# tspooner/rl_markets

Measured on AMD Instinct MI355X. Metric: env-steps/sec (whole node) at 65 536 parallel books, higher is better.
Workload: dtype f64

## Files before the change

rl_markets_amd/csrc/lob_engine.hip:

```cpp
#define LOB_TU_SPLIT 1
#define LOB_TU_MAIN 1
#include <hip/hip_runtime.h>
#include <math.h>
#include <stdio.h>
#include <stdlib.h>
#include <string.h>

#include <algorithm>
#include <climits>
#include <condition_variable>
#include <initializer_list>
#include <map>
#include <mutex>
#include <string>
#include <system_error>
#include <thread>
#include <vector>

#include "lob_internal.h"
#include "lob_fast.h"
#include "lob_kernels.h"
#include "lob_launch.h"

#define HIPCHK(expr)                                                                         \
// ... 375 lines not shown
    int ndev = 0;
    if (hipGetDeviceCount(&ndev) != hipSuccess || ndev < 1 || device < 0 || device >= ndev) {
        lob_set_error("lob_create: no usable HIP device (the engine has no CPU fallback)");
        return LOB_ENODEV;
    }
    HIPCHK(hipSetDevice(device));
    lob_engine* e = new lob_engine();
    e->device = device;
    e->B = n_books;
    e->params = *p;
    e->sw = read_switches();
    {
        hipDeviceProp_t prop;
        if (hipGetDeviceProperties(&prop, device) == hipSuccess && prop.multiProcessorCount > 0) e->n_cus = prop.multiProcessorCount;
    }
#define HIPCHK_E(expr)                                                                       \
    do {                                                                                     \
        hipError_t _e = (expr);                                                              \
        if (_e != hipSuccess) {                                                              \
            lob_set_error(std::string(#expr) + ": " + hipGetErrorString(_e));                \
            lob_destroy(e);                                                                  \
            return LOB_EHIP;                                                                 \
        }                                                                                    \
    } while (0)
    HIPCHK_E(hipStreamCreate(&e->stream));
    HIPCHK_E(hipStreamCreate(&e->stream2));
    HIPCHK_E(hipEventCreateWithFlags(&e->ev_fork, hipEventDisableTiming | hipEventDisableSystemFence));
    HIPCHK_E(hipEventCreateWithFlags(&e->ev_join, hipEventDisableTiming | hipEventDisableSystemFence));
    HIPCHK_E(hipEventCreateWithFlags(&e->ev_stagger, hipEventDisableTiming | hipEventDisableSystemFence));
    HIPCHK_E(hipEventCreateWithFlags(&e->ev_rest_go, hipEventDisableTiming | hipEventDisableSystemFence));
    HIPCHK_E(hipEventCreateWithFlags(&e->ev_rest_done, hipEventDisableTiming | hipEventDisableSystemFence));
    if (hipHostMalloc((void**)&e->rest_hint, LOB_HINT_RING * sizeof(u64), hipHostMallocMapped) == hipSuccess) {
        memset(e->rest_hint, 0, LOB_HINT_RING * sizeof(u64));
        if (hipHostGetDevicePointer((void**)&e->rest_hint_dev, e->rest_hint, 0) != hipSuccess) e->rest_hint_dev = nullptr;
    } else e->rest_hint = nullptr;
    if (!e->rest_hint_dev && e->rest_hint) { hipHostFree(e->rest_hint); e->rest_hint = nullptr; }
    for (int i = 0; i < LOB_HINT_RING && e->rest_hint; i++) HIPCHK_E(hipEventCreateWithFlags(&e->hint_ev[i], hipEventDisableTiming));

    DevParams& P = e->P;
    memset(&P, 0, sizeof P);
    P.D = p->depth; P.T = p->max_trades; P.W = lob_rec_words(p->depth, p->max_trades); P.Wd = drec_words(p->depth, p->max_trades); P.V = p->n_vars;
    for (int i = 0; i < LOB_MAX_VARS; i++) P.vars[i] = p->vars[i];
    lobh::TickTable tt;
    lobh::build_tick_table(p->market, tt);
    P.n_bands = tt.n;
    for (int i = 0; i < LOB_MAX_BANDS; i++) { P.band_lb[i] = tt.lb[i]; P.band_tick[i] = tt.tick[i]; P.band_cum[i] = tt.cum[i]; P.band_pt[i] = tt.pt[i]; P.band_pp[i] = tt.pp[i]; }
    P.open_ms = p->market.open_ms; P.close_ms = p->market.close_ms;
    P.order_size = p->order_size; P.reward_measure = p->reward_measure;
    P.pos_lb = p->pos_lb; P.pos_ub = p->pos_ub;
    P.damping_factor = p->damping_factor; P.pos_weight = p->pos_weight; P.trd_weight = p->trd_weight; P.pnl_weight = p->pnl_weight;
    P.target_price = p->target_price; P.quote_mode = p->quote_mode;
    P.ewma_alpha = 2.0 / ((double)(size_t)p->lb_rsi + 1.0);
    P.M = p->memory_size;
    P.w0 = p->group_weights[0]; P.w1 = p->group_weights[1]; P.w2 = p->group_weights[2];
    P.gamma = p->gamma; P.alpha = p->alpha; P.epsilon = p->epsilon;
    P.policy = p->policy; P.tau = p->tau; P.beta = p->beta;
    P.trace_rate = trace_rate;
    for (int k = 0; k <= LOB_TRACE_GENS; k++) P.trace_pow[k] = trace_pow[k];
    P.trace_kmax = trace_kmax;
    P.trace_gens = P.trace_kmax <= 32 ? 32 : LOB_TRACE_GENS;
    P.r_learn = p->algo >= LOB_ALGO_R_LEARN;
    P.algo = p->algo == LOB_ALGO_R_LEARN ? LOB_ALGO_QLAMBDA : p->algo == LOB_ALGO_ONLINE_R_LEARN ? LOB_ALGO_SARSA
             : p->algo == LOB_ALGO_DOUBLE_R_LEARN ? LOB_ALGO_DOUBLE_Q : p->algo;
    P.theta_private = p->theta_mode == LOB_THETA_PRIVATE;
    e->plan = plan_paths(P, n_books, e->n_cus, e->sw);
    P.combine = e->plan.combine;
    P.memo = e->plan.memo;
    P.carry_verdicts = e->plan.carry_verdicts;
    P.sarsa_lanes = e->plan.sarsa_lanes;
    P.epi_epoch = 0;
    P.seed = p->seed; P.book_id_offset = p->book_id_offset;
    P.exp_learn_first = e->sw.exp_learn_first ? 1 : 0;

    DevState& S = e->S;
    memset(&S, 0, sizeof S);
    const size_t B = (size_t)n_books;
    S.B = n_books; S.D = P.D; S.T = P.T; S.W = P.W;
    int rc = LOB_OK;
    auto alloc = [&](auto* ptr, size_t count) { if (rc == LOB_OK) rc = dev_alloc(e, ptr, count); };
#define X(t, n) alloc(&S.n, B);
    LOB_ENV_FIELDS(X)
#undef X
    alloc(&S.hdr, B);
    auto alloc_rm = [&](RMPtrs& r, int w) {
        r.w = w;
        alloc(&r.ring, B * w); alloc(&r.cnt, B); alloc(&r.head, B); alloc(&r.sum, B); alloc(&r.mean, B); alloc(&r.s, B);
    };
    auto alloc_acc = [&](AccPtrs& r, int w) {
        r.w = w;
        alloc(&r.ring, B * w); alloc(&r.cnt, B); alloc(&r.head, B); alloc(&r.sum, B);
    };
    alloc_rm(S.f_midprice, p->lb_mpm);
    alloc_rm(S.f_volatility, p->lb_vlt);
    alloc_rm(S.f_ask_tx, p->lb_svl);
    alloc_rm(S.f_bid_tx, p->lb_svl);
    alloc_rm(S.spread_window, p->lb_spread);
    alloc_rm(S.pnl_ups, p->lb_pnl);
    alloc_rm(S.pnl_downs, p->lb_pnl);
    alloc_rm(S.tp_mp, p->lb_target);
    alloc_acc(S.f_vwap_numer, p->lb_vwap);
    alloc_acc(S.f_vwap_denom, p->lb_vwap);
    alloc(&S.meta, B); alloc(&S.prep, B); alloc(&S.ewma_up, B); alloc(&S.ewma_down, B); alloc(&S.tp_val, B); alloc(&S.persist, B * LOB_PERSIST_N);
    alloc(&S.k_stop, B); alloc(&S.vars, B * 3 * 16); alloc(&S.qs_last, B * LOB_N_ACTIONS); alloc(&S.tr_idx, B * (size_t)P.trace_gens * 32);
    alloc(&S.tr_alive, B * (size_t)P.trace_gens); alloc(&S.theta, (size_t)P.M * (P.theta_private ? B : 1));
    alloc(&S.theta_nz, LOB_NZ_NWORDS(P.M) * (P.theta_private ? B : 1));
    if (P.algo == LOB_ALGO_DOUBLE_Q) {
        alloc(&S.theta_b, (size_t)P.M * (P.theta_private ? B : 1)); alloc(&S.theta_b_nz, LOB_NZ_NWORDS(P.M) * (P.theta_private ? B : 1));
        alloc(&S.qs_last_b, B * LOB_N_ACTIONS); alloc(&S.mt_state, B * LOB_MT_N); alloc(&S.mt_idx, B);
    }
    {
        const bool rl = P.r_learn != 0;
        const size_t nr = rl ? (P.theta_private ? B : 1) : 1;
        alloc(&S.rho, nr); alloc(&S.rho_inc, nr); alloc(&S.rho_cnt, nr); alloc(&S.rl_t, rl ? B : 1);
    }
    alloc(&S.tr_sig, B * (size_t)P.trace_gens * 4); alloc(&S.tr_cbslot, B * (size_t)P.trace_gens);
    {
        int slots = 2048;
        while ((size_t)slots < 8 * B && slots < (1 << 22)) slots <<= 1;
        if (e->sw.cb_slots) slots = e->sw.cb_slots;
        S.cb_slots = slots;
        alloc(&S.cb_key, (size_t)slots); alloc(&S.cb_ident, (size_t)slots * 8);
        S.cb_reps = e->sw.acc_reps ? e->sw.acc_reps : P.memo ? 8 : 1;
        alloc(&S.cb_acc, (size_t)S.cb_reps * slots * 2); alloc(&S.cb_touch, (size_t)slots); alloc(&S.cb_list, 2 * (size_t)slots);
        S.cb_segs = std::min(2048, slots / 4);
        alloc(&S.cb_count, 2 * (size_t)S.cb_segs);
        if (rc == LOB_OK && hipMemsetAsync(S.cb_key, 0xff, (size_t)slots * 8, e->stream) != hipSuccess) rc = LOB_EHIP;
        if (e->plan.dense_ids) {
            alloc(&S.cb_dense, (size_t)slots); alloc(&S.cb_free, (size_t)LOB_CBD_CAP); alloc(&S.cb_free_n, 16);
            alloc(&S.tr_cbd, B * (size_t)P.trace_gens); alloc(&S.cb_part, (size_t)LOB_ACD_MAX_BLOCKS * LOB_CBD_CAP);
            alloc(&S.cb_red, (size_t)LOB_ACD_GROUPS * LOB_CBD_CAP);
            if (rc == LOB_OK && hipMemsetAsync(S.cb_dense, 0xff, (size_t)slots * 4, e->stream) != hipSuccess) rc = LOB_EHIP;
            if (rc == LOB_OK && hipMemsetAsync(S.tr_cbd, 0xff, B * (size_t)P.trace_gens * 8, e->stream) != hipSuccess) rc = LOB_EHIP;
            if (rc == LOB_OK) {
                std::vector<i32> fl(LOB_CBD_CAP), fn(16);
                const int per = LOB_CBD_CAP / 8;
                int have = per;
                if (e->sw.cbd_ids) have = e->sw.cbd_ids / 8;
                S.cb_ids = have * 8;
                for (int x = 0; x < 8; x++) {
                    for (int i = 0; i < have; i++) fl[(size_t)x * per + i] = (have - 1 - i) * 8 + x;
                    fn[2 * x] = have;
                    fn[2 * x + 1] = have;
                }
                if (hipMemcpyAsync(S.cb_free, fl.data(), fl.size() * 4, hipMemcpyHostToDevice, e->stream) != hipSuccess ||
                    hipMemcpyAsync(S.cb_free_n, fn.data(), fn.size() * 4, hipMemcpyHostToDevice, e->stream) != hipSuccess ||
                    hipStreamSynchronize(e->stream) != hipSuccess) rc = LOB_EHIP;
            }
            if (rc == LOB_OK && hipFuncSetAttribute((const void*)accumulate_dense_kernel, hipFuncAttributeMaxDynamicSharedMemorySize, (int)acd_lds_bytes()) != hipSuccess) {
                lob_set_error("hipFuncSetAttribute(accumulate_dense_kernel: dynamic LDS)");
                rc = LOB_EHIP;
            }
        }
    }
    {
        S.mk_slots = 1 << 16;
        const size_t ms = (size_t)S.mk_slots;
        alloc(&S.mk_hash, ms); alloc(&S.mk_ident, ms * 4); alloc(&S.mk_stamp, ms); alloc(&S.mk_list, 2 * ms); alloc(&S.mk_count, 2);
        alloc(&S.mk_rec, 2 * ms * LOB_MK_REC);
        if (P.memo && P.algo == LOB_ALGO_DOUBLE_Q) alloc(&S.mk_rec_b, 2 * ms * LOB_MK_REC);
        alloc(&S.mk_tiles, P.memo ? ms * LOB_N_ACTIONS * 32 : 1); alloc(&S.mk_tiles_ok, ms); alloc(&S.mk_marked, ms); alloc(&S.mk_marklist, ms);
        alloc(&S.mk_markcount, 1); alloc(&S.tr_list, B); alloc(&S.tr_list_n, 2); alloc(&S.tr_list2, B); alloc(&S.tr_list2_n, 2);
        alloc(&S.acc_list, B); alloc(&S.acc_list_n, 2); alloc(&S.acc_pend, B); alloc(&S.dir_list, P.combine ? B * (size_t)P.trace_gens : 1);
        alloc(&S.dir_list_n, 2); alloc(&S.mk_slot, B); alloc(&S.mk_slot_last, B);
        if (rc == LOB_OK && hipMemsetAsync(S.mk_hash, 0xff, ms * 8, e->stream) != hipSuccess) rc = LOB_EHIP;
        if (rc == LOB_OK && hipMemsetAsync(S.mk_slot, 0xff, B * 4, e->stream) != hipSuccess) rc = LOB_EHIP;
        if (rc == LOB_OK && hipMemsetAsync(S.mk_slot_last, 0xff, B * 4, e->stream) != hipSuccess) rc = LOB_EHIP;
        const bool sl = P.sarsa_lanes != 0;
        S.ow_slots = sl ? 1 << 25 : 1;
        S.amb_cap = sl ? (int)std::min<long long>((long long)P.M, 1 << 18) : 1;
        if (sl && e->sw.ow_slots) S.ow_slots = e->sw.ow_slots;
        if (sl && e->sw.amb_cap) S.amb_cap = e->sw.amb_cap;
        alloc(&S.tr_mslot, sl ? B * (size_t)P.trace_gens : 1); alloc(&S.ow_tab, (size_t)S.ow_slots);
        alloc(&S.amb_bits, sl ? (size_t)P.M / 32 + 1 : 1); alloc(&S.amb_new, 2 * (size_t)S.amb_cap); alloc(&S.amb_new_n, 2); alloc(&S.amb_flag, 1);
        alloc(&S.mk_amb, sl ? ms * LOB_N_ACTIONS : 1); alloc(&S.mk_all, sl ? ms : 1); alloc(&S.mk_all_n, 1);
        if (rc == LOB_OK && hipMemsetAsync(S.tr_mslot, 0xff, (sl ? B * (size_t)P.trace_gens : 1) * 4, e->stream) != hipSuccess) rc = LOB_EHIP;
        if (rc == LOB_OK && hipMemsetAsync(S.ow_tab, 0xff, (size_t)S.ow_slots * 8, e->stream) != hipSuccess) rc = LOB_EHIP;
    }
    {
        int cs = 5;
        while ((((size_t)P.M >> cs) + 31) / 32 > 20480) cs++;
        P.cshift = cs;
        const size_t cwords = (((size_t)P.M >> cs) + 32) / 32;
        P.cwords4 = (int)((cwords + 3) / 4);
        alloc(&S.theta_nzx, P.memo ? (size_t)P.M / 32 + 1 : 1); alloc(&S.theta_nzc, (size_t)P.cwords4 * 4);
// ... 1711 lines not shown
```

rl_markets_amd/csrc/lob_env.h:

```cpp
#ifndef LOB_ENV_H
#define LOB_ENV_H

#include <hip/hip_runtime.h>

#include "lob_internal.h"
#include "lob_state.h"

LOB_HD int drec_pad4(int n) { return (n + 3) & ~3; }
LOB_HD int drec_words(int D, int T) { return 4 + 4 * drec_pad4(D) + drec_pad4(2 * T); }
LOB_HD int drec_ask_px(int, int) { return 4; }
LOB_HD int drec_ask_vol(int D, int) { return 4 + drec_pad4(D); }
LOB_HD int drec_bid_px(int D, int) { return 4 + 2 * drec_pad4(D); }
LOB_HD int drec_bid_vol(int D, int) { return 4 + 3 * drec_pad4(D); }
LOB_HD int drec_trades(int D, int) { return 4 + 4 * drec_pad4(D); }
LOB_HD void drec_from_abi(const uint32_t* src, int D, int T, uint32_t* dst) {
    const int Wd = drec_words(D, T);
    for (int i = 0; i < Wd; i++) dst[i] = 0;
    dst[0] = src[LOB_REC_TIME];
    dst[1] = src[LOB_REC_FLAGS];
    for (int l = 0; l < D; l++) {
        dst[drec_ask_px(D, T) + l] = src[lob_rec_ask_px(D, T) + l];
        dst[drec_ask_vol(D, T) + l] = src[lob_rec_ask_vol(D, T) + l];
        dst[drec_bid_px(D, T) + l] = src[lob_rec_bid_px(D, T) + l];
        dst[drec_bid_vol(D, T) + l] = src[lob_rec_bid_vol(D, T) + l];
// ... 1412 lines not shown

__device__ inline void persist_io(const DevState& S, int b, bool save) {
    int i = 0;
    const int B = S.B;
#define X(n)                                                                                   \
    if (save) { S.persist[(size_t)(i + 0) * B + b] = S.n.sum[b]; S.persist[(size_t)(i + 1) * B + b] = S.n.mean[b]; S.persist[(size_t)(i + 2) * B + b] = S.n.s[b]; } \
    else { S.n.sum[b] = S.persist[(size_t)(i + 0) * B + b]; S.n.mean[b] = S.persist[(size_t)(i + 1) * B + b]; S.n.s[b] = S.persist[(size_t)(i + 2) * B + b]; }   \
    i += 3;
    X(f_midprice) X(f_volatility) X(f_ask_tx) X(f_bid_tx) X(spread_window) X(tp_mp)
#undef X
#define X(n)                                                            \
    if (save) S.persist[(size_t)i * B + b] = S.n.sum[b];                \
    else S.n.sum[b] = S.persist[(size_t)i * B + b];                     \
    i += 1;
    X(f_vwap_numer) X(f_vwap_denom)
#undef X
    if (save) {
        S.persist[(size_t)(i + 0) * B + b] = S.ewma_up[b];
        S.persist[(size_t)(i + 1) * B + b] = S.ewma_down[b];
        S.persist[(size_t)(i + 2) * B + b] = S.tp_val[b];
    } else {
        S.ewma_up[b] = S.persist[(size_t)(i + 0) * B + b];
        S.ewma_down[b] = S.persist[(size_t)(i + 1) * B + b];
        S.tp_val[b] = S.persist[(size_t)(i + 2) * B + b];
    }
}

__device__ inline void prepass_begin(const EnvCtx& c, PrepState& st, BookMeta& M) {
    const DevParams& P = c.P;
    const DevState& S = c.S;
    const int b = c.b;
    MarketR m;
    m.cursor = 0; m.time_ms = 0; m.rec_cur = -1; m.rec_last = -1;
    m.ap0 = m.bp0 = m.lap0 = m.lbp0 = 0.0;
    m.a_tv = m.b_tv = 0;
    m.a_obsval = m.b_obsval = 0.0; m.a_obsvol = m.b_obsvol = 0;
    m.ewma_up = S.ewma_up[b]; m.ewma_down = S.ewma_down[b]; m.tp_val = S.tp_val[b];
    m.records = 0;
#define X(n) S.n.cnt[b] = 0;
    LOB_ROLLING_MEANS(X)
    LOB_ACCUMULATORS(X)
#undef X
    M.n_track = 0; M.k_warm = -1; M.init_ok = 0; M.complete = 0; M._pad = 0;
    M.ex_first = -1; M.ex_cur = -1; M.ex_last = -1; M.ex_time = 0; M.ex_records = 0;
    bool ok = true;
    while (ok && !is_open(P, m.time_ms)) ok = mk_update_book_profiles(c, m);
    M.rec_cur0 = m.rec_cur; M.rec_last0 = m.rec_last; M.time0 = m.time_ms;
    M.mid0 = (m.ap0 + m.bp0) / 2.0; M.mid_prev0 = (m.lap0 + m.lbp0) / 2.0;
    if (!ok) { M.ex_cur = m.rec_cur; M.ex_last = m.rec_last; M.ex_time = m.time_ms; M.complete = 1; }
    st.cursor = m.cursor; st.time_ms = m.time_ms; st.rec_cur = m.rec_cur; st.rec_last = m.rec_last;
    st.ap0 = m.ap0; st.bp0 = m.bp0; st.lap0 = m.lap0; st.lbp0 = m.lbp0;
    st.a_tv = m.a_tv; st.b_tv = m.b_tv;
    st.ewma_up = m.ewma_up; st.ewma_down = m.ewma_down; st.tp_val = m.tp_val;
    st.records = m.records;
    st.k = 0;
    st.prev_first = m.rec_cur;
}

__device__ inline void prepass_begin_books(const EnvCtx& c, PrepState& st, BookMeta& M) {
    const DevParams& P = c.P;
    MarketR m;
    m.cursor = 0; m.time_ms = 0; m.rec_cur = -1; m.rec_last = -1;
    m.ap0 = m.bp0 = m.lap0 = m.lbp0 = 0.0;
    m.a_tv = m.b_tv = 0;
    m.a_obsval = m.b_obsval = 0.0; m.a_obsvol = m.b_obsvol = 0;
    m.ewma_up = m.ewma_down = m.tp_val = 0.0;
    m.records = 0;
    M.n_track = 0; M.k_warm = -1; M.init_ok = 0; M.complete = 0; M._pad = 0;
    M.ex_first = -1; M.ex_cur = -1; M.ex_last = -1; M.ex_time = 0; M.ex_records = 0;
    bool ok = true;
    while (ok && !is_open(P, m.time_ms)) ok = mk_update_book_profiles(c, m);
    M.rec_cur0 = m.rec_cur; M.rec_last0 = m.rec_last; M.time0 = m.time_ms;
    M.mid0 = (m.ap0 + m.bp0) / 2.0; M.mid_prev0 = (m.lap0 + m.lbp0) / 2.0;
    if (!ok) { M.ex_cur = m.rec_cur; M.ex_last = m.rec_last; M.ex_time = m.time_ms; M.complete = 1; }
    st.cursor = m.cursor; st.time_ms = m.time_ms; st.rec_cur = m.rec_cur; st.rec_last = m.rec_last;
    st.ap0 = m.ap0; st.bp0 = m.bp0; st.lap0 = m.lap0; st.lbp0 = m.lbp0;
    st.a_tv = m.a_tv; st.b_tv = m.b_tv;
    st.ewma_up = st.ewma_down = st.tp_val = 0.0;
    st.records = m.records;
    st.k = 0;
    st.prev_first = m.rec_cur;
}

template <int TM>
__device__ inline void prepass_run(const EnvCtx& c, PrepState& st, BookMeta& M, int k_stop, bool write_track) {
    const DevParams& P = c.P;
    const DevState& S = c.S;
    const int b = c.b, B = S.B;
    MarketR m;
    m.cursor = st.cursor; m.time_ms = st.time_ms; m.rec_cur = st.rec_cur; m.rec_last = st.rec_last;
    m.ap0 = st.ap0; m.bp0 = st.bp0; m.lap0 = st.lap0; m.lbp0 = st.lbp0;
    m.a_tv = st.a_tv; m.b_tv = st.b_tv;
    m.a_obsval = m.b_obsval = 0.0; m.a_obsvol = m.b_obsvol = 0;
    m.ewma_up = st.ewma_up; m.ewma_down = st.ewma_down; m.tp_val = st.tp_val;
    m.records = st.records;
    int k = st.k;
    int prev_first = st.prev_first;
    RMReg w_mid, w_vol, w_spr, w_tp, w_atx, w_btx;
    AccReg w_vn, w_vd;
    rm_load(S.f_midprice, b, w_mid); rm_load(S.f_volatility, b, w_vol); rm_load(S.spread_window, b, w_spr);
    rm_load(S.tp_mp, b, w_tp); rm_load(S.f_ask_tx, b, w_atx); rm_load(S.f_bid_tx, b, w_btx);
    acc_load(S.f_vwap_numer, b, w_vn); acc_load(S.f_vwap_denom, b, w_vd);
#ifndef LOB_PRE_TOUCH
#define LOB_PRE_TOUCH 0
#endif
#if LOB_PRE_TOUCH
    PreRow<TM> R0;
    uint32_t nt[4] = {0u, 0u, 0u, 0u};
#else
    PreRow<TM> R0, R1;
#endif
    i32 t1 = 0, t2 = 0;
    bool piped = false;
    int band_px = 0, band_tk = 0;
    rm_prep(S.f_midprice, B, b, w_mid); rm_prep(S.f_volatility, B, b, w_vol); rm_prep(S.spread_window, B, b, w_spr);
    rm_prep(S.tp_mp, B, b, w_tp); rm_prep(S.f_ask_tx, B, b, w_atx); rm_prep(S.f_bid_tx, B, b, w_btx);
    acc_prep(S.f_vwap_numer, B, b, w_vn); acc_prep(S.f_vwap_denom, B, b, w_vd);
    while (!M.complete && k < k_stop) {
        const int first = m.cursor;
#if LOB_PRE_TOUCH
        {
            const int last = c.n_ev() - 1;
            const uint32_t* r2 = c.row(first + 2 < last ? first + 2 : last);
            const int wl = P.Wd - 1;
            nt[0] = r2[0]; nt[1] = r2[16 < wl ? 16 : wl]; nt[2] = r2[32 < wl ? 32 : wl]; nt[3] = r2[wl];
        }
        pre_row_issue<TM>(c, first, R0);
        if (!piped) t1 = pre_row_time(c, first + 1);
#else
        if (!piped) { pre_row_issue<TM>(c, first, R0); t1 = pre_row_time(c, first + 1); }
        pre_row_issue<TM>(c, first + 1, R1);
        t2 = pre_row_time(c, first + 2);
#endif
        if (first < c.n_ev() && (R0.hdr.y & LOB_EVT_FLAG_TAS_DRY)) {
            M.ex_first = -1; M.ex_cur = m.rec_cur; M.ex_last = m.rec_last; M.ex_time = m.time_ms; M.ex_records = 0;
            M.complete = 1;
            break;
        }
        f64 tp[TM];
        i64 tv[TM];
        if (prev_first + 1 == first) {
#pragma unroll
            for (int i = 0; i < TM; i++) { tp[i] = 0.0; tv[i] = 0; }
            int ntr = 0;
            merge_trade_slots<TM>(c, R0.tr, ntr, tp, tv);
        } else {
            load_trades<TM>(c, prev_first + 1, first, tp, tv);
        }
        prev_first = first;
        const f64 mp = (m.ap0 + m.bp0) / 2.0;
        m.a_obsval = 0.0; m.a_obsvol = 0; m.b_obsval = 0.0; m.b_obsvol = 0;
#pragma unroll
        for (int i = 0; i < TM; i++) {
            if (i >= P.T || tv[i] <= 0) continue;
            if (tp[i] < mp) continue;
            m.a_obsval += tp[i] * (f64)tv[i];
            m.a_obsvol += tv[i];
        }
#pragma unroll
        for (int ii = 0; ii < TM; ii++) {
            const int i = TM - 1 - ii;
            if (i >= P.T || tv[i] <= 0) continue;
            if (tp[i] > mp) continue;
            m.b_obsval += tp[i] * (f64)tv[i];
            m.b_obsvol += tv[i];
        }
        const i64 rec0 = m.records;
        if (!mk_update_book_profiles_pre<TM>(c, m, R0, t1)) {
            M.ex_first = first; M.ex_cur = m.rec_cur; M.ex_last = m.rec_last; M.ex_time = m.time_ms;
            M.ex_records = m.records - rec0;
            M.complete = 1;
            break;
        }
        if (m.lap0 == 0.0 || m.lbp0 == 0.0) c.err(LOB_ERR_UNDEF_PRICE);
        const f64 mid = (m.ap0 + m.bp0) / 2.0, lmid = (m.lap0 + m.lbp0) / 2.0;
        const int tick_ap0 = lobh::to_ticks_hint((*c.tk), m.ap0, band_px), tick_bp0 = lobh::to_ticks_hint((*c.tk), m.bp0, band_px);
        const i64 mpt = (i64)lobh::to_ticks_hint((*c.tk), mid, band_px);
        const f64 mpm = mid - lmid, sp = m.ap0 - m.bp0;
        rm_apply_reg(S.f_midprice, B, b, w_mid, (f64)mpt);
        rm_apply_reg(S.f_volatility, B, b, w_vol, (f64)mpt);
        acc_apply_reg(S.f_vwap_numer, B, b, w_vn, m.a_obsval + m.b_obsval);
        acc_apply_reg(S.f_vwap_denom, B, b, w_vd, (f64)(m.a_obsvol + m.b_obsvol));
        rm_apply_reg(S.spread_window, B, b, w_spr, 0.0 > sp ? 0.0 : sp);
        f64 micro;
        {
            f64 div = (f64)(m.a_tv + m.b_tv);
            f64 mpm_a = (f64)m.a_tv * m.bp0, mpm_b = m.ap0 * (f64)m.b_tv;
            micro = (mpm_a + mpm_b) / div;
        }
        rm_apply_reg(S.tp_mp, B, b, w_tp, P.target_price == LOB_TP_MICROPRICE ? micro : mid);
        m.tp_val = w_tp.mean;
        {
            f64 up = 0.0 > mpm ? 0.0 : mpm;
            f64 dn = fabs(0.0 < mpm ? 0.0 : mpm);
            m.ewma_up = (P.ewma_alpha * up) + ((1 - P.ewma_alpha) * m.ewma_up);
            m.ewma_down = (P.ewma_alpha * dn) + ((1 - P.ewma_alpha) * m.ewma_down);
        }
        rm_apply_reg(S.f_ask_tx, B, b, w_atx, (f64)m.a_obsvol);
        rm_apply_reg(S.f_bid_tx, B, b, w_btx, (f64)m.b_obsvol);
        rm_prep(S.f_midprice, B, b, w_mid); rm_prep(S.f_volatility, B, b, w_vol); rm_prep(S.spread_window, B, b, w_spr);
        rm_prep(S.tp_mp, B, b, w_tp); rm_prep(S.f_ask_tx, B, b, w_atx); rm_prep(S.f_bid_tx, B, b, w_btx);
        acc_prep(S.f_vwap_numer, B, b, w_vn); acc_prep(S.f_vwap_denom, B, b, w_vd);

        if (write_track) {
            Track t;
            t.rec_first = first; t.rec_last = m.rec_cur; t.time_ms = m.time_ms;
            t.tick_ap0 = tick_ap0; t.tick_bp0 = tick_bp0;
            {
                int ntr = 0;
#pragma unroll
                for (int i = 0; i < TM; i++) ntr += (i < P.T && tv[i] > 0) ? 1 : 0;
                t.info = (ntr < 2 ? ntr : 2) | (ntr <= 2 ? LOB_TRK_TRADES_OK : 0);
                t.tr_px[0] = (f32)tp[0]; t.tr_vol[0] = tv[0];
                t.tr_px[1] = TM > 1 ? (f32)tp[TM > 1 ? 1 : 0] : 0.0f; t.tr_vol[1] = TM > 1 ? tv[TM > 1 ? 1 : 0] : 0;
                t.bap = (f32)m.ap0; t.bbp = (f32)m.bp0;
            }
            t.mid = mid; t.tp_val = m.tp_val; t.spread_mean = w_spr.mean;
            t.a_tv = m.a_tv; t.b_tv = m.b_tv;
            t.mv[LOB_MV_SPD] = (f32)ulb((f64)(tick_ap0 - tick_bp0), 0.0, 20.0);
            {
                const f64 front = (f64)mpt;
                i32 bi = w_mid.head - w_mid.cnt + 1;
                if (bi < 0) bi += S.f_midprice.w;
                const f64 back = w_mid.cnt == S.f_midprice.w ? w_mid.old : S.f_midprice.ring[(size_t)bi * B + b];
                t.mv[LOB_MV_MPM] = (f32)ulb((f64)(lobh::to_ticks_hint((*c.tk), front, band_tk) - lobh::to_ticks_hint((*c.tk), back, band_tk)), -10.0, 10.0);
            }
            {
                f64 v_a = (f64)m.a_tv, v_b = (f64)m.b_tv;
                t.mv[LOB_MV_IMB] = (f32)((v_a + v_b) > 0 ? 5 * (v_b - v_a) / (v_b + v_a) : 0.0);
                f64 q_a = w_atx.sum, q_b = w_btx.sum;
                t.mv[LOB_MV_SVL] = (f32)((q_a + q_b) > 0 ? 5 * (q_b - q_a) / (q_a + q_b) : 0.0);
            }
            {
                f64 var = w_vol.s / (f64)(w_vol.cnt - 1);
                f64 sd = var > 0 ? sqrt(var) : 0.0;
                t.mv[LOB_MV_VOL] = (f32)ulb(5.0 * sd, 0.0, 10.0);
                f64 u = m.ewma_up, d = m.ewma_down;
                t.mv[LOB_MV_RSI] = (f32)((u + d) != 0.0 ? 5.0 * (u - d) / (u + d) : 0.0);
                f64 vw = w_vn.sum / w_vd.sum;
                t.mv[LOB_MV_VWAP] = (f32)ulb(vw / w_spr.mean, -10.0, 10.0);
                t.mv[7] = 0.0f;
            }
            c.track_w(k) = t;
            if (M.k_warm < 0 && w_atx.cnt == S.f_ask_tx.w && w_btx.cnt == S.f_bid_tx.w && w_vn.cnt == S.f_vwap_numer.w &&
                w_vd.cnt == S.f_vwap_denom.w && w_vol.cnt == S.f_volatility.w && w_mid.cnt == S.f_midprice.w &&
                w_tp.cnt == S.tp_mp.w && w_spr.cnt == S.spread_window.w)
                M.k_warm = k + 1;
        }
        if (k + 1 == M.k_warm) prev_first = m.rec_cur;
        k++;
        piped = m.cursor == first + 1;
#if LOB_PRE_TOUCH
        t2 = (i32)nt[0];
        asm volatile("" ::"v"(nt[1]), "v"(nt[2]), "v"(nt[3]));
        if (piped) t1 = t2;
#else
        if (piped) { R0 = R1; t1 = t2; }
#endif
    }
    rm_store(S.f_midprice, b, w_mid); rm_store(S.f_volatility, b, w_vol); rm_store(S.spread_window, b, w_spr);
    rm_store(S.tp_mp, b, w_tp); rm_store(S.f_ask_tx, b, w_atx); rm_store(S.f_bid_tx, b, w_btx);
    acc_store(S.f_vwap_numer, b, w_vn); acc_store(S.f_vwap_denom, b, w_vd);
    st.cursor = m.cursor; st.time_ms = m.time_ms; st.rec_cur = m.rec_cur; st.rec_last = m.rec_last;
    st.ap0 = m.ap0; st.bp0 = m.bp0; st.lap0 = m.lap0; st.lbp0 = m.lbp0;
    st.a_tv = m.a_tv; st.b_tv = m.b_tv;
    st.ewma_up = m.ewma_up; st.ewma_down = m.ewma_down; st.tp_val = m.tp_val;
    st.records = m.records;
    st.k = k;
    st.prev_first = prev_first;
    S.ewma_up[b] = m.ewma_up; S.ewma_down[b] = m.ewma_down; S.tp_val[b] = m.tp_val;
    if (write_track) {
        M.n_track = k;
        M.init_ok = M.k_warm > 0 ? 1 : 0;
    }
}


__device__ inline void lds_block_barrier() {
    __builtin_amdgcn_fence(__ATOMIC_RELEASE, "workgroup", "local");
    __builtin_amdgcn_s_barrier();
    __builtin_amdgcn_fence(__ATOMIC_ACQUIRE, "workgroup", "local");
}
struct PreXch {
    i64 mpt[64], a_obsvol[64], b_obsvol[64], a_tv[64], b_tv[64];
    f64 sp[64], mpm[64], tp_in[64], obsval[64];
    i32 spd[64], live[64];
    i32 go, _pad;
};
template <int TM>
__device__ inline void prepass_books_role(const DevParams* Pp, const DevState* Sp, int b, const uint32_t* rows, const TickLds* tk, PrepState* stp, BookMeta* Mp,
                                                int k_stop, bool on, PreXch* xch, int lane) {
    const DevParams& P = *Pp;
    const DevState& S = *Sp;
    const EnvCtx c(P, S, b, tk, rows);
    PrepState& st = *stp;
    BookMeta& M = *Mp;
    MarketR m;
    m.cursor = st.cursor; m.time_ms = st.time_ms; m.rec_cur = st.rec_cur; m.rec_last = st.rec_last;
    m.ap0 = st.ap0; m.bp0 = st.bp0; m.lap0 = st.lap0; m.lbp0 = st.lbp0;
    m.a_tv = st.a_tv; m.b_tv = st.b_tv;
    m.a_obsval = m.b_obsval = 0.0; m.a_obsvol = m.b_obsvol = 0;
    m.ewma_up = m.ewma_down = m.tp_val = 0.0;
    m.records = st.records;
    int k = st.k;
    int prev_first = st.prev_first;
    PreRow<TM> R0;
    uint32_t nt[4] = {0u, 0u, 0u, 0u};
    i32 t1 = 0;
    bool piped = false;
    int band_px = 0;
    int w_max = S.f_midprice.w;
    {
        const int ws[] = {S.f_volatility.w, S.f_ask_tx.w, S.f_bid_tx.w, S.spread_window.w, S.tp_mp.w, S.f_vwap_numer.w, S.f_vwap_denom.w};
        for (int w : ws) w_max = w > w_max ? w : w_max;
    }
#pragma unroll 1
    for (int it = 0;; it++) {
        PreXch& X = xch[it & 1];
        int live = 0;
        if (on && !M.complete && k < k_stop) {
            do {
                const int first = m.cursor;
                {
                    const int last = c.n_ev() - 1;
                    const uint32_t* r2 = c.row(first + 2 < last ? first + 2 : last);
                    const int wl = P.Wd - 1;
                    nt[0] = r2[0]; nt[1] = r2[16 < wl ? 16 : wl]; nt[2] = r2[32 < wl ? 32 : wl]; nt[3] = r2[wl];
                }
                pre_row_issue<TM>(c, first, R0);
                if (!piped) t1 = pre_row_time(c, first + 1);
                if (first < c.n_ev() && (R0.hdr.y & LOB_EVT_FLAG_TAS_DRY)) {
                    M.ex_first = -1; M.ex_cur = m.rec_cur; M.ex_last = m.rec_last; M.ex_time = m.time_ms; M.ex_records = 0;
                    M.complete = 1;
                    break;
                }
                f64 tp[TM];
                i64 tv[TM];
                if (prev_first + 1 == first) {
#pragma unroll
                    for (int i = 0; i < TM; i++) { tp[i] = 0.0; tv[i] = 0; }
                    int ntr = 0;
                    merge_trade_slots<TM>(c, R0.tr, ntr, tp, tv);
                } else {
                    load_trades<TM>(c, prev_first + 1, first, tp, tv);
                }
// ... 174 lines not shown
```

rl_markets_amd/csrc/lob_state.h:

```cpp
#ifndef LOB_STATE_H
#define LOB_STATE_H

#include <stdint.h>

#include "../../include/lob_engine.h"

typedef long long i64;
typedef unsigned long long u64;
typedef int i32;
typedef double f64;
typedef float f32;

#if defined(__HIP_DEVICE_COMPILE__)
template <class T> __device__ __forceinline__ T* lob_g(T* p) {
    return (T*)(__attribute__((address_space(1))) T*)(unsigned long long)p;
}
#else
template <class T> inline T* lob_g(T* p) { return p; }
#endif

template <class T> struct GP {
    T* p;
    __host__ __device__ __forceinline__ operator T*() const { return lob_g(p); }
    __host__ __device__ __forceinline__ T* operator->() const { return lob_g(p); }
// ... 103 lines not shown
    f64 ap0, bp0, lap0, lbp0;
    i64 a_tv, b_tv;
    f64 ewma_up, ewma_down, tp_val;
    i64 records;
    i32 k;
    i32 prev_first;
};

struct __attribute__((aligned(64))) LHdr {
    i32 done;
    i32 time_ms;
    i32 slot_cur;
    i32 zero_mask;
    i32 action;
    i32 stepped;
    i32 tr_head;
    i32 tr_n;
    u64 rng_ctr;
    f64 reward;
    f64 td;
    f64 upd;
};

#define LOB_CBD_CAP 16384
#define LOB_ACD_MAX_BLOCKS 256
#define LOB_ACD_MARK 0x7ff4000000000001ull
#define LOB_ML_BLOCKS 256
#define LOB_ML_ROWS 8192
#define LOB_PERSIST_N 32
#define LOB_PROF_N 32
#define LOB_MK_REC 10
#define LOB_MK_PROBES 16
#define LOB_HL_CAP 23
#define LOB_HL_ROW 24
#define LOB_HL_MAX 35
#define LOB_HL_REC 36
#define LOB_VD_STRIDE 72
#define LOB_NZ_SHIFT 3
#define LOB_NZ_WORD(i) ((i) >> (LOB_NZ_SHIFT + 5))
#define LOB_NZ_BIT(i) (1u << (((i) >> LOB_NZ_SHIFT) & 31))
#define LOB_NZ_NWORDS(M) ((((size_t)(M) >> LOB_NZ_SHIFT) >> 5) + 1)
#define LOB_NZ_WORDS 256
#define LOB_NZ_FILTER 128
#define LOB_NZ_NEW_MAX 256

struct RMPtrs {
    GP<f64> ring;
    GP<i32> cnt;
    GP<i32> head;
    GP<f64> sum;
    GP<f64> mean;
    GP<f64> s;
    i32 w;
};
struct AccPtrs {
    GP<f64> ring;
    GP<i32> cnt;
    GP<i32> head;
    GP<f64> sum;
    i32 w;
};

struct DevState {
    i32 B;
    i32 D, T, W;
    i32 n_events;
    GP<const uint32_t> records;
    GP<const i64> rec_phase;
    GP<const i32> rec_len;
    __device__ __forceinline__ i32 events_of(int b) const { return rec_len ? rec_len[b] : n_events; }

#define X(t, n) GP<t> n;
    LOB_ENV_FIELDS(X)
#undef X
#define X(n) RMPtrs n;
    LOB_ROLLING_MEANS(X)
#undef X
#define X(n) AccPtrs n;
    LOB_ACCUMULATORS(X)
#undef X

    GP<Track> track;
    i32 track_len, track_mask;
    GP<BookMeta> meta;
    GP<PrepState> prep;
    GP<f64> ewma_up;
    GP<f64> ewma_down;
    GP<f64> tp_val;
    GP<f64> persist;
    GP<i32> k_stop;

    GP<LHdr> hdr;
    GP<f32> vars;
    GP<f64> qs_last;
    GP<i32> tr_idx;
    GP<uint32_t> tr_alive;

    GP<f64> theta;
    GP<f64> theta_b;
    GP<uint32_t> theta_b_nz;
    GP<f64> qs_last_b;
    GP<u64> mt_state;
    GP<i32> mt_idx;
    GP<i32> tr_sig;
    GP<i32> tr_cbslot;
    GP<i32> tr_mslot;
    GP<u64> cb_key;
    GP<i32> cb_ident;
    GP<f64> cb_acc;
    GP<uint32_t> cb_touch;
    GP<i32> cb_list;
    GP<i32> cb_count;
    i32 cb_slots;
    i32 cb_reps;
    i32 cb_segs;
    i32 cb_par;
    GP<i32> cb_dense;
    GP<i32> cb_free;
    GP<i32> cb_free_n;
    GP<u64> tr_cbd;
    GP<f64> cb_part;
    GP<f64> cb_red;
    i32 cb_ids;
    i32 cb_dense_on;
    GP<uint16_t> verdict;
    GP<uint16_t> verdict_b;
    GP<i32> nz_new;
    GP<i32> nz_epoch;
    GP<uint32_t> theta_nz;
    GP<u64> mk_hash;
    GP<i32> mk_ident;
    GP<i32> mk_stamp;
    GP<i32> mk_list;
    GP<i32> mk_count;
    GP<f64> mk_rec;
    GP<f64> mk_rec_b;
    GP<i32> mk_tiles;
    GP<i32> mk_tiles_ok;
    GP<uint32_t> mk_marked;
    GP<i32> mk_marklist;
    GP<i32> mk_markcount;
    GP<u64> ow_tab;
    i32 ow_slots;
    GP<uint32_t> amb_bits;
    GP<i32> amb_new;
    GP<i32> amb_new_n;
    i32 amb_cap;
    GP<i32> amb_flag;
    GP<uint32_t> mk_amb;
    GP<i32> mk_all;
    GP<i32> mk_all_n;
    GP<i32> mk_slot;
    GP<i32> mk_slot_last;
    i32 mk_slots;
    GP<uint32_t> theta_nzx;
    GP<uint32_t> theta_nzc;
    GP<uint32_t> theta_nzd;
    GP<const uint32_t> nzd_terms;
    GP<i32> tr_list;
    GP<i32> tr_list_n;
    GP<i32> tr_list2;
    GP<i32> tr_list2_n;
    GP<i32> acc_list;
    GP<i32> acc_list_n;
    GP<uint8_t> acc_pend;
    GP<i32> dir_list;
// ... 89 lines not shown
```

Baseline: 288.9 million.

## Index prepass rolling-window rings by step with power-of-two mask and shared midprice ring

Rolling-window rings used in the prepass are now sized to a common power of two and addressed by step index `k & mask`. This replaces per-window head/count bookkeeping in registers. The volatility window reuses the midprice ring because both push the same value, which removes one ring's storage and writes. Evicted values are prefetched one step ahead, and warm-up is detected with a single comparison against the largest window. Head and count are reconstructed from k only at the end, so any other code that reads these rings with the old head-based layout could disagree.

```diff
diff --git a/rl_markets_amd/csrc/lob_engine.hip b/rl_markets_amd/csrc/lob_engine.hip
--- a/rl_markets_amd/csrc/lob_engine.hip
+++ b/rl_markets_amd/csrc/lob_engine.hip
@@ -481,24 +481,34 @@
     LOB_ENV_FIELDS(X)
 #undef X
     alloc(&S.hdr, B);
-    auto alloc_rm = [&](RMPtrs& r, int w) {
+    int pre_len = 1;
+    for (int w : {p->lb_mpm, p->lb_vlt, p->lb_svl, p->lb_spread, p->lb_target, p->lb_vwap})
+        while (pre_len < w) pre_len *= 2;
+    S.pre_mask = pre_len - 1;
+    auto alloc_rm = [&](RMPtrs& r, int w, int ring_len) {
         r.w = w;
-        alloc(&r.ring, B * w); alloc(&r.cnt, B); alloc(&r.head, B); alloc(&r.sum, B); alloc(&r.mean, B); alloc(&r.s, B);
+        if (ring_len) alloc(&r.ring, B * ring_len);
+        alloc(&r.cnt, B); alloc(&r.head, B); alloc(&r.sum, B); alloc(&r.mean, B); alloc(&r.s, B);
     };
-    auto alloc_acc = [&](AccPtrs& r, int w) {
+    auto alloc_acc = [&](AccPtrs& r, int w, int ring_len) {
         r.w = w;
-        alloc(&r.ring, B * w); alloc(&r.cnt, B); alloc(&r.head, B); alloc(&r.sum, B);
+        alloc(&r.ring, B * ring_len); alloc(&r.cnt, B); alloc(&r.head, B); alloc(&r.sum, B);
     };
-    alloc_rm(S.f_midprice, p->lb_mpm);
-    alloc_rm(S.f_volatility, p->lb_vlt);
-    alloc_rm(S.f_ask_tx, p->lb_svl);
-    alloc_rm(S.f_bid_tx, p->lb_svl);
-    alloc_rm(S.spread_window, p->lb_spread);
-    alloc_rm(S.pnl_ups, p->lb_pnl);
-    alloc_rm(S.pnl_downs, p->lb_pnl);
-    alloc_rm(S.tp_mp, p->lb_target);
-    alloc_acc(S.f_vwap_numer, p->lb_vwap);
-    alloc_acc(S.f_vwap_denom, p->lb_vwap);
+    alloc_rm(S.f_midprice, p->lb_mpm, pre_len);
+#ifdef LOB_EXPERIMENTS
+    alloc_rm(S.f_volatility, p->lb_vlt, pre_len);
+#else
+    alloc_rm(S.f_volatility, p->lb_vlt, 0);
+    S.f_volatility.ring = S.f_midprice.ring.p;
+#endif
+    alloc_rm(S.f_ask_tx, p->lb_svl, pre_len);
+    alloc_rm(S.f_bid_tx, p->lb_svl, pre_len);
+    alloc_rm(S.spread_window, p->lb_spread, pre_len);
+    alloc_rm(S.pnl_ups, p->lb_pnl, p->lb_pnl);
+    alloc_rm(S.pnl_downs, p->lb_pnl, p->lb_pnl);
+    alloc_rm(S.tp_mp, p->lb_target, pre_len);
+    alloc_acc(S.f_vwap_numer, p->lb_vwap, pre_len);
+    alloc_acc(S.f_vwap_denom, p->lb_vwap, pre_len);
     alloc(&S.meta, B); alloc(&S.prep, B); alloc(&S.ewma_up, B); alloc(&S.ewma_down, B); alloc(&S.tp_val, B); alloc(&S.persist, B * LOB_PERSIST_N);
     alloc(&S.k_stop, B); alloc(&S.vars, B * 3 * 16); alloc(&S.qs_last, B * LOB_N_ACTIONS); alloc(&S.tr_idx, B * (size_t)P.trace_gens * 32);
     alloc(&S.tr_alive, B * (size_t)P.trace_gens); alloc(&S.theta, (size_t)P.M * (P.theta_private ? B : 1));
diff --git a/rl_markets_amd/csrc/lob_env.h b/rl_markets_amd/csrc/lob_env.h
--- a/rl_markets_amd/csrc/lob_env.h
+++ b/rl_markets_amd/csrc/lob_env.h
@@ -1518,6 +1518,37 @@
     st.prev_first = m.rec_cur;
 }
 
+struct PreRM { f64 sum, mean, s, old; };
+struct PreAcc { f64 sum, old; };
+__device__ inline size_t pre_slot(int k, int mask, int B) { return (size_t)(k & mask) * B; }
+__device__ inline void pre_rm_load(const RMPtrs& r, int b, PreRM& g) { g.sum = r.sum[b]; g.mean = r.mean[b]; g.s = r.s[b]; g.old = 0.0; }
+__device__ inline void pre_rm_push(PreRM& g, f64 val, int k, int w) {
+    g.sum += val;
+    const f64 n = (f64)((k < w ? k : w) + 1);
+    const f64 old_mean = g.mean;
+    g.mean += (val - g.mean) / n;
+    g.s += (val - g.mean) * (val - old_mean);
+    if (k >= w) {
+        g.sum -= g.old;
+        const f64 n2 = (f64)w;
+        const f64 old_mean2 = g.mean;
+        g.mean -= (g.old - g.mean) / n2;
+        g.s -= (g.old - g.mean) * (g.old - old_mean2);
+    }
+}
+__device__ inline void pre_acc_push(PreAcc& g, f64 val, int k, int w) {
+    g.sum += val;
+    if (k >= w) g.sum -= g.old;
+}
+__device__ inline void pre_cnt_head(i32* cnt, i32* head, int b, int k, int w) {
+    cnt[b] = k < w ? k : w;
+    if (k > 0) head[b] = (k - 1) % w;
+}
+__device__ inline void pre_rm_store(const RMPtrs& r, int b, const PreRM& g, int k) {
+    r.sum[b] = g.sum; r.mean[b] = g.mean; r.s[b] = g.s;
+    pre_cnt_head(r.cnt, r.head, b, k, r.w);
+}
+
 template <int TM>
 __device__ inline void prepass_run(const EnvCtx& c, PrepState& st, BookMeta& M, int k_stop, bool write_track) {
     const DevParams& P = c.P;
@@ -1532,11 +1563,20 @@
     m.records = st.records;
     int k = st.k;
     int prev_first = st.prev_first;
-    RMReg w_mid, w_vol, w_spr, w_tp, w_atx, w_btx;
-    AccReg w_vn, w_vd;
-    rm_load(S.f_midprice, b, w_mid); rm_load(S.f_volatility, b, w_vol); rm_load(S.spread_window, b, w_spr);
-    rm_load(S.tp_mp, b, w_tp); rm_load(S.f_ask_tx, b, w_atx); rm_load(S.f_bid_tx, b, w_btx);
-    acc_load(S.f_vwap_numer, b, w_vn); acc_load(S.f_vwap_denom, b, w_vd);
+    PreRM w_mid, w_vol, w_spr, w_tp, w_atx, w_btx;
+    PreAcc w_vn, w_vd;
+    pre_rm_load(S.f_midprice, b, w_mid); pre_rm_load(S.f_volatility, b, w_vol); pre_rm_load(S.spread_window, b, w_spr);
+    pre_rm_load(S.tp_mp, b, w_tp); pre_rm_load(S.f_ask_tx, b, w_atx); pre_rm_load(S.f_bid_tx, b, w_btx);
+    w_vn.sum = S.f_vwap_numer.sum[b]; w_vd.sum = S.f_vwap_denom.sum[b];
+    const int pm = S.pre_mask;
+    f64* const r_px = S.f_midprice.ring + b; f64* const r_spr = S.spread_window.ring + b; f64* const r_tp = S.tp_mp.ring + b;
+    f64* const r_atx = S.f_ask_tx.ring + b; f64* const r_btx = S.f_bid_tx.ring + b;
+    f64* const r_vn = S.f_vwap_numer.ring + b; f64* const r_vd = S.f_vwap_denom.ring + b;
+    const int wl_mid = S.f_midprice.w, wl_vol = S.f_volatility.w, wl_spr = S.spread_window.w, wl_tp = S.tp_mp.w, wl_svl = S.f_ask_tx.w,
+              wl_vwap = S.f_vwap_numer.w;
+    int w_max = wl_mid;
+    w_max = wl_vol > w_max ? wl_vol : w_max; w_max = wl_spr > w_max ? wl_spr : w_max; w_max = wl_tp > w_max ? wl_tp : w_max;
+    w_max = wl_svl > w_max ? wl_svl : w_max; w_max = wl_vwap > w_max ? wl_vwap : w_max;
 #ifndef LOB_PRE_TOUCH
 #define LOB_PRE_TOUCH 0
 #endif
@@ -1549,9 +1589,13 @@
     i32 t1 = 0, t2 = 0;
     bool piped = false;
     int band_px = 0, band_tk = 0;
-    rm_prep(S.f_midprice, B, b, w_mid); rm_prep(S.f_volatility, B, b, w_vol); rm_prep(S.spread_window, B, b, w_spr);
-    rm_prep(S.tp_mp, B, b, w_tp); rm_prep(S.f_ask_tx, B, b, w_atx); rm_prep(S.f_bid_tx, B, b, w_btx);
-    acc_prep(S.f_vwap_numer, B, b, w_vn); acc_prep(S.f_vwap_denom, B, b, w_vd);
+#define LOB_PRE_FETCH(kk)                                                                                                   \
+    w_mid.old = r_px[pre_slot((kk) - wl_mid, pm, B)]; w_vol.old = r_px[pre_slot((kk) - wl_vol, pm, B)];                        \
+    w_spr.old = r_spr[pre_slot((kk) - wl_spr, pm, B)]; w_tp.old = r_tp[pre_slot((kk) - wl_tp, pm, B)];                         \
+    { const size_t o = pre_slot((kk) - wl_svl, pm, B); w_atx.old = r_atx[o]; w_btx.old = r_btx[o]; }                          \
+    { const size_t o = pre_slot((kk) - wl_vwap, pm, B); w_vn.old = r_vn[o]; w_vd.old = r_vd[o]; }
+    LOB_PRE_FETCH(k)
+    f64 mid_cur = (m.ap0 + m.bp0) / 2.0;
     while (!M.complete && k < k_stop) {
         const int first = m.cursor;
 #if LOB_PRE_TOUCH
@@ -1584,7 +1628,7 @@
             load_trades<TM>(c, prev_first + 1, first, tp, tv);
         }
         prev_first = first;
-        const f64 mp = (m.ap0 + m.bp0) / 2.0;
+        const f64 mp = mid_cur;
         m.a_obsval = 0.0; m.a_obsvol = 0; m.b_obsval = 0.0; m.b_obsvol = 0;
 #pragma unroll
         for (int i = 0; i < TM; i++) {
@@ -1610,21 +1654,24 @@
         }
         if (m.lap0 == 0.0 || m.lbp0 == 0.0) c.err(LOB_ERR_UNDEF_PRICE);
         const f64 mid = (m.ap0 + m.bp0) / 2.0, lmid = (m.lap0 + m.lbp0) / 2.0;
+        mid_cur = mid;
         const int tick_ap0 = lobh::to_ticks_hint((*c.tk), m.ap0, band_px), tick_bp0 = lobh::to_ticks_hint((*c.tk), m.bp0, band_px);
         const i64 mpt = (i64)lobh::to_ticks_hint((*c.tk), mid, band_px);
         const f64 mpm = mid - lmid, sp = m.ap0 - m.bp0;
-        rm_apply_reg(S.f_midprice, B, b, w_mid, (f64)mpt);
-        rm_apply_reg(S.f_volatility, B, b, w_vol, (f64)mpt);
-        acc_apply_reg(S.f_vwap_numer, B, b, w_vn, m.a_obsval + m.b_obsval);
-        acc_apply_reg(S.f_vwap_denom, B, b, w_vd, (f64)(m.a_obsvol + m.b_obsvol));
-        rm_apply_reg(S.spread_window, B, b, w_spr, 0.0 > sp ? 0.0 : sp);
+        const size_t slot = pre_slot(k, pm, B);
+        r_px[slot] = (f64)mpt;
+        pre_rm_push(w_mid, (f64)mpt, k, wl_mid);
+        pre_rm_push(w_vol, (f64)mpt, k, wl_vol);
+        pre_acc_push(w_vn, r_vn[slot] = m.a_obsval + m.b_obsval, k, wl_vwap);
+        pre_acc_push(w_vd, r_vd[slot] = (f64)(m.a_obsvol + m.b_obsvol), k, wl_vwap);
+        pre_rm_push(w_spr, r_spr[slot] = 0.0 > sp ? 0.0 : sp, k, wl_spr);
         f64 micro;
         {
             f64 div = (f64)(m.a_tv + m.b_tv);
             f64 mpm_a = (f64)m.a_tv * m.bp0, mpm_b = m.ap0 * (f64)m.b_tv;
             micro = (mpm_a + mpm_b) / div;
         }
-        rm_apply_reg(S.tp_mp, B, b, w_tp, P.target_price == LOB_TP_MICROPRICE ? micro : mid);
+        pre_rm_push(w_tp, r_tp[slot] = P.target_price == LOB_TP_MICROPRICE ? micro : mid, k, wl_tp);
         m.tp_val = w_tp.mean;
         {
             f64 up = 0.0 > mpm ? 0.0 : mpm;
@@ -1632,11 +1679,9 @@
             m.ewma_up = (P.ewma_alpha * up) + ((1 - P.ewma_alpha) * m.ewma_up);
             m.ewma_down = (P.ewma_alpha * dn) + ((1 - P.ewma_alpha) * m.ewma_down);
         }
-        rm_apply_reg(S.f_ask_tx, B, b, w_atx, (f64)m.a_obsvol);
-        rm_apply_reg(S.f_bid_tx, B, b, w_btx, (f64)m.b_obsvol);
-        rm_prep(S.f_midprice, B, b, w_mid); rm_prep(S.f_volatility, B, b, w_vol); rm_prep(S.spread_window, B, b, w_spr);
-        rm_prep(S.tp_mp, B, b, w_tp); rm_prep(S.f_ask_tx, B, b, w_atx); rm_prep(S.f_bid_tx, B, b, w_btx);
-        acc_prep(S.f_vwap_numer, B, b, w_vn); acc_prep(S.f_vwap_denom, B, b, w_vd);
+        pre_rm_push(w_atx, r_atx[slot] = (f64)m.a_obsvol, k, wl_svl);
+        pre_rm_push(w_btx, r_btx[slot] = (f64)m.b_obsvol, k, wl_svl);
+        LOB_PRE_FETCH(k + 1)
 
         if (write_track) {
             Track t;
@@ -1656,9 +1701,7 @@
             t.mv[LOB_MV_SPD] = (f32)ulb((f64)(tick_ap0 - tick_bp0), 0.0, 20.0);
             {
                 const f64 front = (f64)mpt;
-                i32 bi = w_mid.head - w_mid.cnt + 1;
-                if (bi < 0) bi += S.f_midprice.w;
-                const f64 back = w_mid.cnt == S.f_midprice.w ? w_mid.old : S.f_midprice.ring[(size_t)bi * B + b];
+                const f64 back = k + 1 >= wl_mid ? w_mid.old : r_px[0];
                 t.mv[LOB_MV_MPM] = (f32)ulb((f64)(lobh::to_ticks_hint((*c.tk), front, band_tk) - lobh::to_ticks_hint((*c.tk), back, band_tk)), -10.0, 10.0);
             }
             {
@@ -1668,7 +1711,7 @@
                 t.mv[LOB_MV_SVL] = (f32)((q_a + q_b) > 0 ? 5 * (q_b - q_a) / (q_a + q_b) : 0.0);
             }
             {
-                f64 var = w_vol.s / (f64)(w_vol.cnt - 1);
+                f64 var = w_vol.s / (f64)((k + 1 < wl_vol ? k + 1 : wl_vol) - 1);
                 f64 sd = var > 0 ? sqrt(var) : 0.0;
                 t.mv[LOB_MV_VOL] = (f32)ulb(5.0 * sd, 0.0, 10.0);
                 f64 u = m.ewma_up, d = m.ewma_down;
@@ -1678,10 +1721,7 @@
                 t.mv[7] = 0.0f;
             }
             c.track_w(k) = t;
-            if (M.k_warm < 0 && w_atx.cnt == S.f_ask_tx.w && w_btx.cnt == S.f_bid_tx.w && w_vn.cnt == S.f_vwap_numer.w &&
-                w_vd.cnt == S.f_vwap_denom.w && w_vol.cnt == S.f_volatility.w && w_mid.cnt == S.f_midprice.w &&
-                w_tp.cnt == S.tp_mp.w && w_spr.cnt == S.spread_window.w)
-                M.k_warm = k + 1;
+            if (M.k_warm < 0 && k + 1 >= w_max) M.k_warm = k + 1;
         }
         if (k + 1 == M.k_warm) prev_first = m.rec_cur;
         k++;
@@ -1694,9 +1734,11 @@
         if (piped) { R0 = R1; t1 = t2; }
 #endif
     }
-    rm_store(S.f_midprice, b, w_mid); rm_store(S.f_volatility, b, w_vol); rm_store(S.spread_window, b, w_spr);
-    rm_store(S.tp_mp, b, w_tp); rm_store(S.f_ask_tx, b, w_atx); rm_store(S.f_bid_tx, b, w_btx);
-    acc_store(S.f_vwap_numer, b, w_vn); acc_store(S.f_vwap_denom, b, w_vd);
+#undef LOB_PRE_FETCH
+    pre_rm_store(S.f_midprice, b, w_mid, k); pre_rm_store(S.f_volatility, b, w_vol, k); pre_rm_store(S.spread_window, b, w_spr, k);
+    pre_rm_store(S.tp_mp, b, w_tp, k); pre_rm_store(S.f_ask_tx, b, w_atx, k); pre_rm_store(S.f_bid_tx, b, w_btx, k);
+    S.f_vwap_numer.sum[b] = w_vn.sum; S.f_vwap_denom.sum[b] = w_vd.sum;
+    pre_cnt_head(S.f_vwap_numer.cnt, S.f_vwap_numer.head, b, k, wl_vwap); pre_cnt_head(S.f_vwap_denom.cnt, S.f_vwap_denom.head, b, k, wl_vwap);
     st.cursor = m.cursor; st.time_ms = m.time_ms; st.rec_cur = m.rec_cur; st.rec_last = m.rec_last;
     st.ap0 = m.ap0; st.bp0 = m.bp0; st.lap0 = m.lap0; st.lbp0 = m.lbp0;
     st.a_tv = m.a_tv; st.b_tv = m.b_tv;
diff --git a/rl_markets_amd/csrc/lob_state.h b/rl_markets_amd/csrc/lob_state.h
--- a/rl_markets_amd/csrc/lob_state.h
+++ b/rl_markets_amd/csrc/lob_state.h
@@ -209,6 +209,7 @@
 
     GP<Track> track;
     i32 track_len, track_mask;
+    i32 pre_mask;
     GP<BookMeta> meta;
     GP<PrepState> prep;
     GP<f64> ewma_up;
```

Result: no change. 286.5 million (-0.8%).
